# UbiquityRobotics/fiducials

Hardware: NVIDIA H100
Metric: frames/sec 1920x1080 (detect+pose) (higher is better)
Workload: dtype u8/i32 (threshold, contours), f32/f64 (sub-pixel, pose, map)

## Files before the change

fiducials_b200/csrc/fid_map.cu:

```cuda
#include <cuda_runtime.h>
#include <stdio.h>
#include <string.h>

#include <algorithm>
#include <vector>

#include "../../include/fiducials_b200.h"
#include "slam.cuh"

using namespace fid;



#include "fid_map_internal.h"

struct SeqArgs {
    MapState* state;
    MapEntry* entries;
    uint32_t* links;
    int cap, links_wpr;
    int32_t* hash;
    int hash_size;
    int n_instances, n_msgs;
    const int32_t* offsets;
    const Obs* obs;
    double* var_scratch;
    int* slot_scratch;
    const Twv* tf;
    int have_base_cam, have_cam_base;
    double weighting_scale, systematic_error;
    int use_area;
    RobotPose* robot;
};

__global__ void k_map_sequence(const SeqArgs a) {
    const int inst = blockIdx.x * blockDim.x + threadIdx.x;
    if (inst >= a.n_instances) return;
    MapState st = a.state[inst];
    MapEntry* e = a.entries + (size_t)inst * a.cap;
    uint32_t* links = a.links ? a.links + (size_t)inst * a.cap * a.links_wpr : nullptr;
    const int32_t* off = a.offsets + (size_t)inst * (a.n_msgs + 1);
    MapHash hash{a.hash + (size_t)inst * 2 * a.hash_size, a.hash + (size_t)inst * 2 * a.hash_size + a.hash_size, a.hash_size};
    for (int k = 0; k < a.n_msgs; k++) {
        RobotPose rp;
        map_update(st, e, links, a.obs + off[k], off[k + 1] - off[k], a.have_base_cam ? &a.tf[0] : nullptr, a.have_cam_base ? &a.tf[1] : nullptr, a.weighting_scale,
                   a.use_area, a.systematic_error, &rp, &hash, a.var_scratch + off[k], a.slot_scratch + off[k]);
        if (a.robot) a.robot[(size_t)inst * a.n_msgs + k] = rp;
    }
    a.state[inst] = st;
}

__global__ void k_map_export(const MapState* state, const MapEntry* entries, int cap, int inst, fid_map_record* table) {
    const MapState st = state[inst];
    const MapEntry* e = entries + (size_t)inst * cap;
    for (int i = threadIdx.x; i < cap; i += blockDim.x) {
        fid_map_record r;
        r.fiducial_id = -1;
        r.num_obs = 0;
        r.t[0] = r.t[1] = r.t[2] = 0;
        r.q[0] = r.q[1] = r.q[2] = 0;
        r.q[3] = 1;
        r.variance = 0;
        if (i < st.n) {
            int rank = 0;
            for (int j = 0; j < st.n; j++) rank += e[j].id < e[i].id ? 1 : 0;
            r.fiducial_id = e[i].id;
            r.num_obs = e[i].num_obs;
            r.t[0] = e[i].pose.t[0];
            r.t[1] = e[i].pose.t[1];
            r.t[2] = e[i].pose.t[2];
            m_to_q(e[i].pose.R, r.q);
            r.variance = e[i].pose.var;
            table[rank] = r;
        }
        if (i >= st.n) table[i] = r;
    }
}

#define MERGE_MAX_KEYS 4096
__device__ __forceinline__ int merge_key(int id) { return id < 0 ? 0x7fffffff : id; }
__device__ int table_find(const fid_map_record* tab, int cap, int id) {
    int lo = 0, hi = cap;
    while (lo < hi) {
        const int mid = (lo + hi) >> 1;
        if (merge_key(tab[mid].fiducial_id) < id)
            lo = mid + 1;
        else
            hi = mid;
    }
    return (lo < cap && tab[lo].fiducial_id == id) ? lo : -1;
}
__device__ void merge_fold(const fid_map_record* tables, int cap, int n_tables, int t0, int i0, MapEntry* out) {
    const fid_map_record& r0 = tables[(size_t)t0 * cap + i0];
    Twv pose;
    q_to_m(r0.q, pose.R);
    pose.t[0] = r0.t[0];
    pose.t[1] = r0.t[1];
    pose.t[2] = r0.t[2];
    pose.var = r0.variance;
    int num = r0.num_obs;
    for (int t = t0 + 1; t < n_tables; t++) {
        const fid_map_record* tab = tables + (size_t)t * cap;
        const int j = table_find(tab, cap, r0.fiducial_id);
        if (j < 0) continue;
        num += tab[j].num_obs;
        if (pose.var == 0.0) continue;
        Twv other;
        q_to_m(tab[j].q, other.R);
        other.t[0] = tab[j].t[0];
        other.t[1] = tab[j].t[1];
        other.t[2] = tab[j].t[2];
        other.var = tab[j].variance;
        if (other.var == 0.0)
            pose = other;
        else
            twv_update(pose, other);
    }
    out->id = r0.fiducial_id;
    out->num_obs = num;
    out->pose = pose;
}

struct MergedHeader {
    int32_t n;
    int32_t overflow;
};

__global__ void __launch_bounds__(1024) k_map_merge_view(int cap, int n_tables, const fid_map_record* tables, MapEntry* merged, MergedHeader* hdr) {
    __shared__ unsigned long long keys[MERGE_MAX_KEYS];
    const int total = n_tables * cap;
    for (int e = threadIdx.x; e < MERGE_MAX_KEYS; e += blockDim.x) {
        unsigned long long k = ~0ull;
        if (e < total) {
            const int t = e / cap, i = e - t * cap;
            const int id = tables[e].fiducial_id;
            bool owner = id >= 0;
            for (int t2 = 0; owner && t2 < t; t2++) owner = table_find(tables + (size_t)t2 * cap, cap, id) < 0;
            if (owner) k = ((unsigned long long)(unsigned int)id << 32) | (unsigned int)e;
            (void)i;
        }
        keys[e] = k;
    }
    __syncthreads();
    for (int k = 2; k <= MERGE_MAX_KEYS; k <<= 1)
        for (int j = k >> 1; j > 0; j >>= 1) {
            for (int e = threadIdx.x; e < MERGE_MAX_KEYS; e += blockDim.x) {
                const int p = e ^ j;
                if (p > e) {
                    const unsigned long long a = keys[e], b = keys[p];
                    const bool up = (e & k) == 0;
                    if ((a > b) == up) {
                        keys[e] = b;
                        keys[p] = a;
                    }
                }
            }
            __syncthreads();
        }
    for (int e = threadIdx.x; e < MERGE_MAX_KEYS; e += blockDim.x) {
        const unsigned long long k = keys[e];
        const bool valid = k != ~0ull;
        if (valid && e < cap) {
            const int src = (int)(unsigned int)k;
            merge_fold(tables, cap, n_tables, src / cap, src % cap, &merged[e]);
        }
        const bool last = valid && (e + 1 == MERGE_MAX_KEYS || keys[e + 1] == ~0ull);
        if (last) {
            hdr->n = e + 1 < cap ? e + 1 : cap;
            hdr->overflow = e + 1 > cap ? 1 : 0;
        }
        if (e == 0 && !valid) {
            hdr->n = 0;
            hdr->overflow = 0;
        }
    }
}

__global__ void k_map_merge_view_serial(int cap, int n_tables, const fid_map_record* tables, MapEntry* merged, MergedHeader* hdr) {
    if (threadIdx.x != 0 || blockIdx.x != 0) return;
    int n = 0, overflow = 0;
    int last_id = -1;
    for (;;) {
        int best = 0x7fffffff, bt = -1, bi = -1;
        for (int t = 0; t < n_tables; t++) {
            const fid_map_record* tab = tables + (size_t)t * cap;
            int lo = 0, hi = cap;
            while (lo < hi) {
                const int mid = (lo + hi) >> 1;
                if (merge_key(tab[mid].fiducial_id) <= last_id)
                    lo = mid + 1;
                else
                    hi = mid;
            }
            if (lo < cap && tab[lo].fiducial_id >= 0 && tab[lo].fiducial_id < best) {
                best = tab[lo].fiducial_id;
                bt = t;
                bi = lo;
            }
        }
        if (bt < 0) break;
        if (n < cap)
            merge_fold(tables, cap, n_tables, bt, bi, &merged[n++]);
// ... 96 lines not shown
extern "C" int fid_map_clear(fid_map* m, int instance) {
    if (!m || instance < 0 || instance >= m->p.n_instances) return FID_ERR_INVALID_ARG;
    CK(cudaSetDevice(m->device));
    CK(cudaStreamSynchronize(m->stream));
    MapState st;
    CK(cudaMemcpy(&st, m->d_state + instance, sizeof(st), cudaMemcpyDeviceToHost));
    st.n = 0;
    st.initial_frame_num = st.frame_num;
    st.origin_fid = -1;
    st.initializing = 0;
    st.overflow = 0;
    st.hash_valid = 0;
    CK(cudaMemcpy(m->d_state + instance, &st, sizeof(st), cudaMemcpyHostToDevice));
    const size_t wpr = (m->p.max_fiducials + 31) / 32;
    CK(cudaMemset(m->d_links + (size_t)instance * m->p.max_fiducials * wpr, 0, sizeof(uint32_t) * (size_t)m->p.max_fiducials * wpr));
    return FID_OK;
}

extern "C" int fid_map_add_fiducial(fid_map* m, int instance, int fiducial_id, const fid_tf* T_mapBase) {
    if (!m || instance < 0 || instance >= m->p.n_instances || fiducial_id < 0) return FID_ERR_INVALID_ARG;
    CK(cudaSetDevice(m->device));
    CK(cudaStreamSynchronize(m->stream));
    MapState st;
    CK(cudaMemcpy(&st, m->d_state + instance, sizeof(st), cudaMemcpyDeviceToHost));
    st.fiducial_to_add = fiducial_id;
    st.add_have_map_base = T_mapBase ? 1 : 0;
    if (T_mapBase) {
        for (int k = 0; k < 3; k++) st.add_map_base[k] = T_mapBase->t[k];
        for (int k = 0; k < 4; k++) st.add_map_base[3 + k] = T_mapBase->q[k];
    }
    CK(cudaMemcpy(m->d_state + instance, &st, sizeof(st), cudaMemcpyHostToDevice));
    return FID_OK;
}

static void tf_to_twv(const fid_tf& t, Twv* o) {
    q_to_m(t.q, o->R);
    o->t[0] = t.t[0];
    o->t[1] = t.t[1];
    o->t[2] = t.t[2];
    o->var = 0.0;
}

extern "C" int fid_map_load(fid_map* m, int instance, int n, const fid_map_file_entry* entries) {
    if (!m || instance < 0 || instance >= m->p.n_instances || n < 0 || (n > 0 && !entries)) return FID_ERR_INVALID_ARG;
    CK(cudaSetDevice(m->device));
    CK(cudaStreamSynchronize(m->stream));
    MapState st;
    CK(cudaMemcpy(&st, m->d_state + instance, sizeof(st), cudaMemcpyDeviceToHost));
    std::vector<MapEntry> e(st.capacity);
    if (st.n) CK(cudaMemcpy(e.data(), m->d_entries + (size_t)instance * st.capacity, sizeof(MapEntry) * st.n, cudaMemcpyDeviceToHost));
    const int lcap = m->p.max_fiducials, lwpr = (lcap + 31) / 32;
    std::vector<uint32_t> rows;
    bool rows_dirty = false;
    const double d2r = 3.14159265358979323846 / 180.0;
    for (int i = 0; i < n; i++) {
        const double hr = entries[i].roll_deg * d2r * 0.5, hp = entries[i].pitch_deg * d2r * 0.5, hy = entries[i].yaw_deg * d2r * 0.5;
        const double cy = cos(hy), sy = sin(hy), cp = cos(hp), sp = sin(hp), cr = cos(hr), sr = sin(hr);
        const double q[4] = {sr * cp * cy - cr * sp * sy, cr * sp * cy + sr * cp * sy, cr * cp * sy - sr * sp * cy, cr * cp * cy + sr * sp * sy};
        int slot = -1;
        for (int j = 0; j < st.n; j++)
            if (e[j].id == entries[i].fiducial_id) slot = j;
        if (slot < 0) {
            if (st.n >= st.capacity) return FID_ERR_CAPACITY;
            slot = st.n++;
        } else {
            if (rows.empty()) {
                rows.resize((size_t)lcap * lwpr);
                CK(cudaMemcpy(rows.data(), m->d_links + (size_t)instance * lcap * lwpr, sizeof(uint32_t) * rows.size(), cudaMemcpyDeviceToHost));
            }
            for (int w = 0; w < lwpr; w++) rows[(size_t)slot * lwpr + w] = 0;
            for (int j = 0; j < lcap; j++) rows[(size_t)j * lwpr + (slot >> 5)] &= ~(1u << (slot & 31));
            rows_dirty = true;
        }
        e[slot].id = entries[i].fiducial_id;
        e[slot].num_obs = entries[i].num_obs;
        q_to_m(q, e[slot].pose.R);
        e[slot].pose.t[0] = entries[i].x;
        e[slot].pose.t[1] = entries[i].y;
        e[slot].pose.t[2] = entries[i].z;
        e[slot].pose.var = entries[i].variance;
    }
    st.hash_valid = 0;
    if (st.n) CK(cudaMemcpy(m->d_entries + (size_t)instance * st.capacity, e.data(), sizeof(MapEntry) * st.n, cudaMemcpyHostToDevice));
    if (rows_dirty) CK(cudaMemcpy(m->d_links + (size_t)instance * lcap * lwpr, rows.data(), sizeof(uint32_t) * rows.size(), cudaMemcpyHostToDevice));
    CK(cudaMemcpy(m->d_state + instance, &st, sizeof(st), cudaMemcpyHostToDevice));
    return FID_OK;
}

template <class T>
static int ensure(T** p, size_t* cap, size_t need) {
    if (need <= *cap) return FID_OK;
    if (*p) cudaFree(*p);
    *p = nullptr;
    *cap = 0;
    const size_t n = std::max<size_t>(need, 1024);
    if (cudaMalloc((void**)p, sizeof(T) * n) != cudaSuccess) {
        cudaGetLastError();
        return FID_ERR_NO_MEMORY;
    }
    *cap = n;
    return FID_OK;
}

static int run_sequence(fid_map* m, int inst_lo, int n_inst, int n_msgs, const int32_t* offsets, const fid_transform* obs, const fid_tf* T_baseCam,
                        const fid_tf* T_camBase, fid_robot_pose* robot, bool async = false) {
    CK(cudaSetDevice(m->device));
    CK(cudaStreamSynchronize(m->stream));
    const size_t n_off = (size_t)n_inst * (n_msgs + 1);
    size_t total_obs = 0;
    for (size_t i = 0; i < n_off; i++) total_obs = std::max<size_t>(total_obs, (size_t)offsets[i]);
    int rc;
    if ((rc = ensure(&m->d_obs, &m->obs_cap, total_obs + 1)) != FID_OK || (rc = ensure(&m->d_var_scratch, &m->var_cap, total_obs + 1)) != FID_OK ||
        (rc = ensure(&m->d_slot_scratch, &m->slot_cap, total_obs + 1)) != FID_OK || (rc = ensure(&m->d_offsets, &m->off_cap, n_off)) != FID_OK ||
        (rc = ensure(&m->d_robot, &m->robot_cap, (size_t)n_inst * n_msgs + 1)) != FID_OK)
        return rc;
    std::vector<Obs> ho(total_obs);
    for (size_t i = 0; i < total_obs; i++) {
        ho[i].id = obs[i].fiducial_id;
        ho[i].pad = 0;
        for (int k = 0; k < 3; k++) ho[i].t[k] = obs[i].translation[k];
        for (int k = 0; k < 4; k++) ho[i].q[k] = obs[i].rotation[k];
        ho[i].object_error = obs[i].object_error;
        ho[i].area = obs[i].fiducial_area;
    }
    if (total_obs) CK(cudaMemcpyAsync(m->d_obs, ho.data(), sizeof(Obs) * total_obs, cudaMemcpyHostToDevice, m->stream));
    CK(cudaMemcpyAsync(m->d_offsets, offsets, sizeof(int32_t) * n_off, cudaMemcpyHostToDevice, m->stream));
    Twv tf[2];
    memset(tf, 0, sizeof(tf));
    if (T_baseCam) tf_to_twv(*T_baseCam, &tf[0]);
    if (T_camBase) tf_to_twv(*T_camBase, &tf[1]);
    CK(cudaMemcpyAsync(m->d_tf, tf, sizeof(tf), cudaMemcpyHostToDevice, m->stream));
    SeqArgs a{};
    const int cap = m->p.max_fiducials;
    a.state = m->d_state + inst_lo;
    a.entries = m->d_entries + (size_t)inst_lo * cap;
    a.links_wpr = (cap + 31) / 32;
    a.links = m->d_links + (size_t)inst_lo * cap * a.links_wpr;
    a.cap = cap;
    a.hash = m->d_hash + (size_t)inst_lo * 2 * m->hash_size;
    a.hash_size = m->hash_size;
    a.n_instances = n_inst;
    a.n_msgs = n_msgs;
    a.offsets = m->d_offsets;
    a.obs = m->d_obs;
    a.var_scratch = m->d_var_scratch;
    a.slot_scratch = m->d_slot_scratch;
    a.tf = m->d_tf;
    a.have_base_cam = T_baseCam ? 1 : 0;
    a.have_cam_base = T_camBase ? 1 : 0;
    a.weighting_scale = m->p.weighting_scale;
    a.systematic_error = m->p.systematic_error;
    a.use_area = m->p.use_fiducial_area_as_weight;
    a.robot = m->d_robot;
    k_map_sequence<<<(n_inst + 31) / 32, 32, 0, m->stream>>>(a);
    CK(cudaGetLastError());
    if (async) return FID_OK;
    std::vector<RobotPose> hr((size_t)n_inst * n_msgs);
    CK(cudaMemcpyAsync(hr.data(), m->d_robot, sizeof(RobotPose) * hr.size(), cudaMemcpyDeviceToHost, m->stream));
    CK(cudaStreamSynchronize(m->stream));
    if (robot)
        for (size_t i = 0; i < hr.size(); i++) {
            robot[i].valid = hr[i].valid;
            robot[i].n_estimates = hr[i].n_estimates;
            for (int k = 0; k < 3; k++) robot[i].t[k] = hr[i].t[k];
            for (int k = 0; k < 4; k++) robot[i].q[k] = hr[i].q[k];
            robot[i].variance = hr[i].var;
        }
    return FID_OK;
}

extern "C" int fid_map_update(fid_map* m, int instance, int n_obs, const fid_transform* obs, const fid_tf* T_baseCam, const fid_tf* T_camBase, fid_robot_pose* robot) {
    if (!m || instance < 0 || instance >= m->p.n_instances || n_obs < 0 || (n_obs > 0 && !obs)) return FID_ERR_INVALID_ARG;
    const int32_t off[2] = {0, n_obs};
    return run_sequence(m, instance, 1, 1, off, obs, T_baseCam, T_camBase, robot);
}

extern "C" int fid_map_update_sequence(fid_map* m, int n_msgs, const int32_t* offsets, const fid_transform* obs, const fid_tf* T_baseCam, const fid_tf* T_camBase,
                                       fid_robot_pose* robot) {
    if (!m || n_msgs < 1 || !offsets) return FID_ERR_INVALID_ARG;
    const size_t n_off = (size_t)m->p.n_instances * (n_msgs + 1);
    for (size_t i = 0; i + 1 < n_off; i++) {
        if ((i + 1) % (n_msgs + 1) == 0) continue;
        const int d = offsets[i + 1] - offsets[i];
        if (d < 0) return FID_ERR_INVALID_ARG;
    }
    return run_sequence(m, 0, m->p.n_instances, n_msgs, offsets, obs, T_baseCam, T_camBase, robot);
}

static int update_frames_impl(fid_map* m, int instance, int n_frames, const int32_t* counts, const fid_transform* transforms, int max_markers, const fid_tf* T_baseCam,
                              const fid_tf* T_camBase, fid_robot_pose* last_robot, bool async) {
    if (!m || instance < 0 || instance >= m->p.n_instances || n_frames < 1 || !counts || !transforms || max_markers < 1) return FID_ERR_INVALID_ARG;
    std::vector<int32_t> off((size_t)n_frames + 1, 0);
    std::vector<fid_transform> flat;
    for (int f = 0; f < n_frames; f++) {
        const int c = std::min(std::max(counts[f], 0), max_markers);
        off[f] = (int32_t)flat.size();
        flat.insert(flat.end(), transforms + (size_t)f * max_markers, transforms + (size_t)f * max_markers + c);
    }
    off[n_frames] = (int32_t)flat.size();
    std::vector<fid_robot_pose> robots((size_t)n_frames);
    fid_transform dummy{};
    const int rc = run_sequence(m, instance, 1, n_frames, off.data(), flat.empty() ? &dummy : flat.data(), T_baseCam, T_camBase, async ? nullptr : robots.data(), async);
    if (rc == FID_OK && last_robot && !async) *last_robot = robots[(size_t)n_frames - 1];
    return rc;
}

extern "C" int fid_map_update_frames(fid_map* m, int instance, int n_frames, const int32_t* counts, const fid_transform* transforms, int max_markers, const fid_tf* T_baseCam,
                                     const fid_tf* T_camBase, fid_robot_pose* last_robot) {
    return update_frames_impl(m, instance, n_frames, counts, transforms, max_markers, T_baseCam, T_camBase, last_robot, false);
}
extern "C" int fid_map_update_frames_async(fid_map* m, int instance, int n_frames, const int32_t* counts, const fid_transform* transforms, int max_markers,
                                           const fid_tf* T_baseCam, const fid_tf* T_camBase) {
    return update_frames_impl(m, instance, n_frames, counts, transforms, max_markers, T_baseCam, T_camBase, nullptr, true);
}
extern "C" int fid_map_sync(fid_map* m) {
    if (!m) return FID_ERR_INVALID_ARG;
    CK(cudaSetDevice(m->device));
    CK(cudaStreamSynchronize(m->stream));
    return FID_OK;
}

extern "C" int fid_map_entries(fid_map* m, int instance, int max_entries, int* n, fid_map_entry* entries) {
    if (!m || instance < 0 || instance >= m->p.n_instances || !n) return FID_ERR_INVALID_ARG;
    CK(cudaSetDevice(m->device));
    CK(cudaStreamSynchronize(m->stream));
    MapState st;
    CK(cudaMemcpy(&st, m->d_state + instance, sizeof(st), cudaMemcpyDeviceToHost));
    std::vector<MapEntry> e(st.n);
    if (st.n) CK(cudaMemcpy(e.data(), m->d_entries + (size_t)instance * st.capacity, sizeof(MapEntry) * st.n, cudaMemcpyDeviceToHost));
    std::sort(e.begin(), e.end(), [](const MapEntry& a, const MapEntry& b) { return a.id < b.id; });
    *n = st.n;
    if (st.n > max_entries) return FID_ERR_CAPACITY;
    for (int i = 0; i < st.n && entries; i++) {
        entries[i].fiducial_id = e[i].id;
        entries[i].num_obs = e[i].num_obs;
        entries[i].x = e[i].pose.t[0];
        entries[i].y = e[i].pose.t[1];
        entries[i].z = e[i].pose.t[2];
        get_rpy(e[i].pose.R, &entries[i].rx, &entries[i].ry, &entries[i].rz);
        entries[i].variance = e[i].pose.var;
    }
    return st.overflow ? FID_ERR_CAPACITY : FID_OK;
}

extern "C" int fid_map_links(fid_map* m, int instance, int max_pairs, int* n_pairs, int32_t* pairs) {
    if (!m || instance < 0 || instance >= m->p.n_instances || !n_pairs || max_pairs < 0) return FID_ERR_INVALID_ARG;
    CK(cudaSetDevice(m->device));
    CK(cudaStreamSynchronize(m->stream));
    MapState st;
    CK(cudaMemcpy(&st, m->d_state + instance, sizeof(st), cudaMemcpyDeviceToHost));
    const int cap = m->p.max_fiducials, wpr = (cap + 31) / 32;
    std::vector<MapEntry> e(st.n);
    std::vector<uint32_t> rows((size_t)st.n * wpr);
    if (st.n) {
        CK(cudaMemcpy(e.data(), m->d_entries + (size_t)instance * st.capacity, sizeof(MapEntry) * st.n, cudaMemcpyDeviceToHost));
        CK(cudaMemcpy(rows.data(), m->d_links + (size_t)instance * cap * wpr, sizeof(uint32_t) * rows.size(), cudaMemcpyDeviceToHost));
    }
    std::vector<std::pair<int32_t, int32_t>> out;
    for (int i = 0; i < st.n; i++)
        for (int j = 0; j < st.n; j++)
            if ((rows[(size_t)i * wpr + (j >> 5)] >> (j & 31)) & 1u) out.emplace_back(e[i].id, e[j].id);
    std::sort(out.begin(), out.end());
    *n_pairs = (int)out.size();
    if ((int)out.size() > max_pairs) return FID_ERR_CAPACITY;
    for (size_t k = 0; k < out.size() && pairs; k++) {
        pairs[2 * k] = out[k].first;
        pairs[2 * k + 1] = out[k].second;
    }
    return FID_OK;
}

extern "C" int fid_map_add_links(fid_map* m, int instance, int n_pairs, const int32_t* pairs) {
    if (!m || instance < 0 || instance >= m->p.n_instances || n_pairs < 0 || (n_pairs > 0 && !pairs)) return FID_ERR_INVALID_ARG;
    if (n_pairs == 0) return FID_OK;
    CK(cudaSetDevice(m->device));
    CK(cudaStreamSynchronize(m->stream));
    MapState st;
    CK(cudaMemcpy(&st, m->d_state + instance, sizeof(st), cudaMemcpyDeviceToHost));
    const int cap = m->p.max_fiducials, wpr = (cap + 31) / 32;
    std::vector<MapEntry> e(st.n);
    std::vector<uint32_t> rows((size_t)st.n * wpr);
    if (!st.n) return FID_OK;
    CK(cudaMemcpy(e.data(), m->d_entries + (size_t)instance * st.capacity, sizeof(MapEntry) * st.n, cudaMemcpyDeviceToHost));
    CK(cudaMemcpy(rows.data(), m->d_links + (size_t)instance * cap * wpr, sizeof(uint32_t) * rows.size(), cudaMemcpyDeviceToHost));
    auto slot_of = [&](int32_t id) {
        for (int i = 0; i < st.n; i++)
            if (e[i].id == id) return i;
        return -1;
    };
    for (int k = 0; k < n_pairs; k++) {
        const int i = slot_of(pairs[2 * k]), j = slot_of(pairs[2 * k + 1]);
        if (i >= 0 && j >= 0) rows[(size_t)i * wpr + (j >> 5)] |= 1u << (j & 31);
    }
    CK(cudaMemcpy(m->d_links + (size_t)instance * cap * wpr, rows.data(), sizeof(uint32_t) * rows.size(), cudaMemcpyHostToDevice));
    return FID_OK;
}

static int launch_export(fid_map* m, int instance, fid_map_record* dst) {
    k_map_export<<<1, 256, 0, m->stream>>>(m->d_state, m->d_entries, m->p.max_fiducials, instance, dst);
    CK(cudaGetLastError());
    return FID_OK;
}

extern "C" int fid_map_export_device(fid_map* m, int instance, void** device_table, size_t* bytes) {
    if (!m || instance < 0 || instance >= m->p.n_instances || !device_table || !bytes) return FID_ERR_INVALID_ARG;
    CK(cudaSetDevice(m->device));
    fid_map_record* tab = m->d_export + (size_t)instance * m->p.max_fiducials;
// ... 92 lines not shown
```

fiducials_b200/csrc/slam.cuh:

```cuda
#pragma once
#include "common.cuh"

namespace fid {

struct Twv {
    double R[9];
    double t[3];
    double var;
};

FID_HD void q_to_m(const double q[4], double m[9]) {
    const double x = q[0], y = q[1], z = q[2], w = q[3];
    const double d = x * x + y * y + z * z + w * w;
    const double s = 2.0 / d;
    const double xs = x * s, ys = y * s, zs = z * s;
    const double wx = w * xs, wy = w * ys, wz = w * zs;
    const double xx = x * xs, xy = x * ys, xz = x * zs;
    const double yy = y * ys, yz = y * zs, zz = z * zs;
    m[0] = 1.0 - (yy + zz);
    m[1] = xy - wz;
    m[2] = xz + wy;
    m[3] = xy + wz;
    m[4] = 1.0 - (xx + zz);
    m[5] = yz - wx;
    m[6] = xz - wy;
    m[7] = yz + wx;
    m[8] = 1.0 - (xx + yy);
}

FID_HD void m_to_q(const double m[9], double q[4]) {
    const double tr = m[0] + m[4] + m[8];
    if (tr > 0.0) {
        double s = sqrt(tr + 1.0);
        q[3] = s * 0.5;
        s = 0.5 / s;
        q[0] = (m[7] - m[5]) * s;
        q[1] = (m[2] - m[6]) * s;
        q[2] = (m[3] - m[1]) * s;
    } else {
        const int i = m[0] < m[4] ? (m[4] < m[8] ? 2 : 1) : (m[0] < m[8] ? 2 : 0);
        const int j = (i + 1) % 3, k = (i + 2) % 3;
        double s = sqrt(m[i * 3 + i] - m[j * 3 + j] - m[k * 3 + k] + 1.0);
        q[i] = s * 0.5;
        s = 0.5 / s;
        q[3] = (m[k * 3 + j] - m[j * 3 + k]) * s;
        q[j] = (m[j * 3 + i] + m[i * 3 + j]) * s;
        q[k] = (m[k * 3 + i] + m[i * 3 + k]) * s;
    }
}

FID_HD void get_rpy(const double m[9], double* roll, double* pitch, double* yaw) {
    if (fabs(m[6]) >= 1.0) {
        *yaw = 0.0;
        const double delta = atan2(m[7], m[8]);
        if (m[6] < 0) {
            *pitch = 3.14159265358979323846 / 2.0;
            *roll = delta;
        } else {
            *pitch = -3.14159265358979323846 / 2.0;
            *roll = delta;
        }
        return;
    }
    *pitch = -asin(m[6]);
    const double c = cos(*pitch);
    *roll = atan2(m[7] / c, m[8] / c);
    *yaw = atan2(m[3] / c, m[0] / c);
}

FID_HD Twv twv_mul(const Twv& a, const Twv& b) {
    Twv o;
    for (int i = 0; i < 3; i++) {
        for (int j = 0; j < 3; j++) o.R[i * 3 + j] = a.R[i * 3] * b.R[j] + a.R[i * 3 + 1] * b.R[3 + j] + a.R[i * 3 + 2] * b.R[6 + j];
        o.t[i] = (a.R[i * 3] * b.t[0] + a.R[i * 3 + 1] * b.t[1] + a.R[i * 3 + 2] * b.t[2]) + a.t[i];
    }
    o.var = a.var + b.var;
    return o;
}

FID_HD Twv twv_inverse(const Twv& a) {
    Twv o;
    for (int i = 0; i < 3; i++)
        for (int j = 0; j < 3; j++) o.R[i * 3 + j] = a.R[j * 3 + i];
    const double n[3] = {-a.t[0], -a.t[1], -a.t[2]};
    for (int i = 0; i < 3; i++) o.t[i] = o.R[i * 3] * n[0] + o.R[i * 3 + 1] * n[1] + o.R[i * 3 + 2] * n[2];
    o.var = a.var;
    return o;
}

FID_HD double prob_at_point(double x, double u, double var) {
    return (1.0 / (sqrt(var) * sqrt(2.0 * 3.14159265358979323846))) * exp(-((x - u) * (x - u)) / (2.0 * var));
}

FID_HD double normalize_david(double new_mean, double mean1, double var1, double mean2, double var2) {
    const double p1 = prob_at_point(new_mean, mean1, var1);
    const double p2 = prob_at_point(new_mean, mean2, var2);
    const double p = sqrt(p1 * p1 + p2 * p2);
    const double r = 1.0 / (p * sqrt(2.0 * 3.14159265358979323846));
    double nv = r * r;
    nv = nv < 1e3 ? nv : 1e3;
    nv = nv > 1e-8 ? nv : 1e-8;
    return nv;
}

FID_HD void twv_update(Twv& self, const Twv& n) {
    double q1[4], q2[4];
    m_to_q(self.R, q1);
    m_to_q(n.R, q2);
    const double v1 = self.var, v2 = n.var;
    const double p1[3] = {self.t[0], self.t[1], self.t[2]};
    const double k = v1 / (v1 + v2);
    for (int i = 0; i < 3; i++) self.t[i] = p1[i] + k * (n.t[i] - p1[i]);
    const double dot = q1[0] * q2[0] + q1[1] * q2[1] + q1[2] * q2[2] + q1[3] * q2[3];
    const double s = sqrt((q1[0] * q1[0] + q1[1] * q1[1] + q1[2] * q1[2] + q1[3] * q1[3]) * (q2[0] * q2[0] + q2[1] * q2[1] + q2[2] * q2[2] + q2[3] * q2[3]));
    double c = (dot < 0 ? -dot : dot) / s;
    c = c < -1.0 ? -1.0 : (c > 1.0 ? 1.0 : c);
    const double theta = acos(c);
    double q[4];
    if (theta != 0.0) {
        const double d = 1.0 / sin(theta);
        const double s0 = sin((1.0 - k) * theta), s1 = sin(k * theta);
        for (int i = 0; i < 4; i++) q[i] = dot < 0 ? (q1[i] * s0 + -q2[i] * s1) * d : (q1[i] * s0 + q2[i] * s1) * d;
    } else {
        for (int i = 0; i < 4; i++) q[i] = q1[i];
    }
    const double nrm = sqrt(q[0] * q[0] + q[1] * q[1] + q[2] * q[2] + q[3] * q[3]);
    for (int i = 0; i < 4; i++) q[i] /= nrm;
    q_to_m(q, self.R);
    const double d0 = n.t[0] - p1[0], d1 = n.t[1] - p1[1], d2 = n.t[2] - p1[2];
    const double mean2 = sqrt(d0 * d0 + d1 * d1 + d2 * d2);
    const double e0 = self.t[0] - p1[0], e1 = self.t[1] - p1[1], e2 = self.t[2] - p1[2];
    const double mean = sqrt(e0 * e0 + e1 * e1 + e2 * e2);
    self.var = normalize_david(mean, 0.0, v1, mean2, v2);
}

struct MapEntry {
    int32_t id;
    int32_t num_obs;
    Twv pose;
};

struct MapState {
    int32_t n;
    int32_t capacity;
    int32_t frame_num;
    int32_t initial_frame_num;
    int32_t origin_fid;
    int32_t initializing;
    int32_t read_only;
    int32_t overflow;
    int32_t hash_size;
    int32_t hash_valid;
    int32_t fiducial_to_add;
    int32_t add_have_map_base;
    double add_map_base[7];
};

struct MapHash {
    int32_t* keys;
    int32_t* vals;
    int32_t size;
};

FID_HD uint32_t map_hash_of(int id) { return (uint32_t)id * 2654435761u; }

FID_HD void map_hash_insert(const MapHash& h, int id, int slot) {
    uint32_t p = map_hash_of(id) & (uint32_t)(h.size - 1);
    while (h.keys[p] != 0 && h.keys[p] != id + 1) p = (p + 1) & (uint32_t)(h.size - 1);
    h.keys[p] = id + 1;
    h.vals[p] = slot;
}

FID_HD void map_hash_rebuild(const MapHash& h, const struct MapEntry* e, int n);

struct Obs {
    int32_t id;
    int32_t pad;
    double t[3];
    double q[4];
    double object_error;
    double area;
};

struct RobotPose {
    int32_t valid;
    int32_t n_estimates;
    double t[3];
    double q[4];
    double var;
};


FID_HD void map_hash_rebuild(const MapHash& h, const MapEntry* e, int n) {
    for (int i = 0; i < h.size; i++) h.keys[i] = 0;
    for (int i = 0; i < n; i++) map_hash_insert(h, e[i].id, i);
}

FID_HD int map_find(const MapState& st, const MapEntry* e, int id, const MapHash* h = nullptr) {
    if (h && h->size > 0) {
        uint32_t p = map_hash_of(id) & (uint32_t)(h->size - 1);
        while (h->keys[p] != 0) {
            if (h->keys[p] == id + 1) return h->vals[p];
            p = (p + 1) & (uint32_t)(h->size - 1);
        }
        return -1;
    }
    for (int i = 0; i < st.n; i++)
        if (e[i].id == id) return i;
    return -1;
}

FID_HD bool isnan3(const double t[3]) { return t[0] != t[0] || t[1] != t[1] || t[2] != t[2]; }

FID_HD Twv obs_cam_fid(const Obs& o, double weighting_scale, int use_area) {
    Twv t;
    q_to_m(o.q, t.R);
    t.t[0] = o.t[0];
    t.t[1] = o.t[1];
    t.t[2] = o.t[2];
    t.var = use_area ? weighting_scale / o.area : weighting_scale * o.object_error;
    return t;
}

FID_HD void map_update_core(MapState& st, MapEntry* e, uint32_t* links, const Obs* obs_in, int n_obs, const Twv* T_baseCam ,
                            const Twv* T_camBase , double weighting_scale, int use_area, double systematic_error, RobotPose* robot,
                            const MapHash* hash, double* var_scratch, int* slot_scratch) {
    if (hash && hash->size > 0 && !st.hash_valid) {
        map_hash_rebuild(*hash, e, st.n);
        st.hash_valid = 1;
    }
    robot->valid = 0;
    robot->n_estimates = 0;
    st.frame_num++;
    if (n_obs > 0 && st.n == 0) st.initializing = 1;
    if (st.initializing) {
        if (st.n == 0) {
            int idx = -1;
            double smallest = -1.0;
            for (int i = 0; i < n_obs; i++) {
                const double* ct = obs_in[i].t;
                const double d = ct[0] * ct[0] + ct[1] * ct[1] + ct[2] * ct[2];
                if (smallest < 0 || d < smallest) {
                    smallest = d;
                    idx = i;
                }
            }
            if (idx >= 0 && st.capacity > 0) {
                st.origin_fid = obs_in[idx].id;
                const Twv cf = obs_cam_fid(obs_in[idx], weighting_scale, use_area);
                Twv T = cf;
                if (T_baseCam) {
                    T = twv_mul(*T_baseCam, cf);
                    T.var = cf.var;
                }
                e[0].id = obs_in[idx].id;
                e[0].num_obs = 0;
                e[0].pose = T;
                st.n = 1;
                if (hash && hash->size > 0) map_hash_insert(*hash, obs_in[idx].id, 0);
            } else if (idx >= 0) {
                st.overflow = 1;
            }
        } else {
            for (int i = 0; i < n_obs; i++) {
                if (obs_in[i].id == st.origin_fid) {
                    const Twv cf = obs_cam_fid(obs_in[i], weighting_scale, use_area);
                    Twv T = cf;
                    if (T_baseCam) {
                        T = twv_mul(*T_baseCam, cf);
                        T.var = cf.var;
                    }
                    const int slot = map_find(st, e, st.origin_fid, hash);
                    if (slot >= 0) {
                        twv_update(e[slot].pose, T);
                        e[slot].num_obs++;
                    }
                    break;
                }
            }
        }
        if (st.frame_num - st.initial_frame_num > 10 && st.origin_fid != -1) {
            st.initializing = 0;
            const int slot = map_find(st, e, st.origin_fid, hash);
            if (slot >= 0) e[slot].pose.var = 0.0;
        }
        return;
    }
    if (n_obs == 0 || !T_baseCam) return;
    Twv camBase;
    if (T_camBase) {
        camBase = *T_camBase;
        camBase.var = 1.0;
    } else {
        for (int i = 0; i < 9; i++) camBase.R[i] = (i % 4 == 0) ? 1.0 : 0.0;
        camBase.t[0] = camBase.t[1] = camBase.t[2] = 0.0;
        camBase.var = 0.0;
    }
    Twv baseCam = *T_baseCam;
    baseCam.var = 1.0;
    int n_est = 0;
    Twv mapBase;
    for (int i = 0; i < n_obs; i++) {
        const Twv cf = obs_cam_fid(obs_in[i], weighting_scale, use_area);
        var_scratch[i] = cf.var;
        const int slot = map_find(st, e, obs_in[i].id, hash);
        if (slot < 0) continue;
        Twv fidCam = twv_inverse(cf);
        Twv p = twv_mul(e[slot].pose, fidCam);
        p = twv_mul(p, camBase);
        double roll, pitch, yaw;
        get_rpy(p.R, &roll, &pitch, &yaw);
        const double* c = cf.t;
        const double zr = p.t[2] / c[2];
        const double s1 = (zr * zr) * (c[0] * c[0] + c[1] * c[1]);
        const double len2 = p.t[0] * p.t[0] + p.t[1] * p.t[1] + p.t[2] * p.t[2];
        const double sr = sin(roll), spt = sin(pitch);
        const double s2 = len2 * (sr * sr);
        const double s3 = len2 * (spt * spt);
        p.var = s1 + s2 + s3 + systematic_error;
        var_scratch[i] = p.var;
        if (isnan3(p.t)) continue;
        if (n_est == 0) {
            mapBase = p;
        } else {
            twv_update(mapBase, p);
        }
        n_est++;
    }
    if (n_est == 0) return;
    robot->valid = 1;
    robot->n_estimates = n_est;
    robot->t[0] = mapBase.t[0];
    robot->t[1] = mapBase.t[1];
    robot->t[2] = mapBase.t[2];
    m_to_q(mapBase.R, robot->q);
    robot->var = mapBase.var;
    const Twv mapCam = twv_mul(mapBase, baseCam);
    if (n_obs > 1 && !st.read_only) {
        for (int i = 0; i < n_obs; i++) {
            Twv cf = obs_cam_fid(obs_in[i], weighting_scale, use_area);
            cf.var = var_scratch[i];
            const Twv mapFid = twv_mul(mapCam, cf);
            if (isnan3(mapFid.t)) continue;
            int slot = map_find(st, e, obs_in[i].id, hash);
            if (slot < 0) {
                if (st.n >= st.capacity) {
                    st.overflow = 1;
                    continue;
                }
                slot = st.n++;
                e[slot].id = obs_in[i].id;
                e[slot].num_obs = 0;
                e[slot].pose = mapFid;
                if (hash && hash->size > 0) map_hash_insert(*hash, obs_in[i].id, slot);
            }
            if (e[slot].pose.var != 0) {
                twv_update(e[slot].pose, mapFid);
                e[slot].num_obs += 2;
            }
        }
        if (links) {
            const int wpr = (st.capacity + 31) / 32;
            int* slots = slot_scratch;
            for (int i = 0; i < n_obs; i++) slots[i] = map_find(st, e, obs_in[i].id, hash);
            for (int i = 0; i < n_obs; i++) {
                if (slots[i] < 0) continue;
                for (int j = 0; j < n_obs; j++) {
                    if (obs_in[j].id == obs_in[i].id || slots[j] < 0) continue;
                    links[(size_t)slots[i] * wpr + (slots[j] >> 5)] |= 1u << (slots[j] & 31);
                }
            }
        }
    }
}

FID_HD void map_handle_add_fiducial(MapState& st, MapEntry* e, const Obs* obs_in, int n_obs, const Twv* T_baseCam, double weighting_scale, int use_area,
                                    const MapHash* hash) {
    if (st.fiducial_to_add == -1) return;
    if (map_find(st, e, st.fiducial_to_add, hash) >= 0) {
        st.fiducial_to_add = -1;
        return;
    }
    for (int i = 0; i < n_obs; i++) {
        if (obs_in[i].id != st.fiducial_to_add) continue;
        Twv T = obs_cam_fid(obs_in[i], weighting_scale, use_area);
        const double var = T.var;
        if (T_baseCam) T = twv_mul(*T_baseCam, T);
        if (st.add_have_map_base) {
            Twv mb;
            q_to_m(st.add_map_base + 3, mb.R);
            mb.t[0] = st.add_map_base[0];
            mb.t[1] = st.add_map_base[1];
            mb.t[2] = st.add_map_base[2];
            mb.var = 0.0;
            T = twv_mul(mb, T);
        }
        T.var = var;
        if (st.n >= st.capacity) {
            st.overflow = 1;
        } else {
            const int slot = st.n++;
            e[slot].id = obs_in[i].id;
            e[slot].num_obs = 0;
            e[slot].pose = T;
            if (hash && hash->size > 0) map_hash_insert(*hash, obs_in[i].id, slot);
            const int os = st.origin_fid != -1 ? map_find(st, e, st.origin_fid, hash) : -1;
            if (os >= 0) e[os].pose.var = 0.0;
        }
        st.initializing = 0;
        st.fiducial_to_add = -1;
        return;
    }
}

FID_HD void map_update(MapState& st, MapEntry* e, uint32_t* links, const Obs* obs_in, int n_obs, const Twv* T_baseCam ,
                       const Twv* T_camBase , double weighting_scale, int use_area, double systematic_error, RobotPose* robot,
                       const MapHash* hash, double* var_scratch, int* slot_scratch) {
    map_update_core(st, e, links, obs_in, n_obs, T_baseCam, T_camBase, weighting_scale, use_area, systematic_error, robot, hash, var_scratch, slot_scratch);
    map_handle_add_fiducial(st, e, obs_in, n_obs, T_baseCam, weighting_scale, use_area, hash);
}

}
```

Measured before the change: 10840.

## Parallelize map update across a warp per instance with shared state

Switches the map sequence kernel from one thread per map instance to one warp per instance. Per-observation pose estimates, map insertions and link-matrix updates are computed in parallel across lanes, using ballot, match_any and shuffles, and state and link masks are kept in shared memory. The pose fusion is split so quaternions are computed in parallel and only the serial fusion step stays ordered. This trades added warp synchronization and shared-memory use for parallelism on frames with many observations, and the reordered updates risk small numerical differences.

```diff
diff --git a/fiducials_b200/csrc/fid_map.cu b/fiducials_b200/csrc/fid_map.cu
--- a/fiducials_b200/csrc/fid_map.cu
+++ b/fiducials_b200/csrc/fid_map.cu
@@ -31,23 +31,203 @@
     double weighting_scale, systematic_error;
     int use_area;
     RobotPose* robot;
+    int shared_per_warp;
 };
 
+constexpr unsigned FULL_MASK = 0xffffffffu;
+constexpr int MAP_WARPS_PER_BLOCK = 4;
+constexpr size_t MAP_STATE_SHARED = (sizeof(MapState) + 15) & ~(size_t)15;
+
+static size_t map_shared_per_warp(int wpr) { return MAP_STATE_SHARED + ((sizeof(uint32_t) * (2 * (size_t)wpr + 1) + 15) & ~(size_t)15); }
+
+__device__ __forceinline__ double shfl_d(double v, int src) { return __shfl_sync(FULL_MASK, v, src); }
+
+__device__ void warp_update(MapState& st, MapEntry* e, uint32_t* links, int wpr, const Obs* obs, int n_obs, const Twv& T_baseCam, const Twv* T_camBase,
+                            double weighting_scale, int use_area, double systematic_error, RobotPose& robot, const MapHash& hash, double* var_scratch,
+                            int* slot_scratch, uint32_t* mask, uint32_t* words, int* n_words) {
+    const int lane = threadIdx.x & 31;
+    const uint32_t lanes_below = (1u << lane) - 1u;
+    const Twv camBase = map_cam_base(T_camBase);
+    int n_est = 0;
+    Twv mapBase = {};
+    for (int base = 0; base < n_obs; base += 32) {
+        const int i = base + lane;
+        bool valid = false;
+        Twv p = {};
+        double q[4] = {0.0, 0.0, 0.0, 1.0};
+        if (i < n_obs) {
+            const Twv cf = obs_cam_fid(obs[i], weighting_scale, use_area);
+            double var = cf.var;
+            const int slot = map_find(st, e, obs[i].id, &hash);
+            if (slot >= 0) {
+                p = map_pose_estimate(cf, e[slot].pose, camBase, systematic_error);
+                var = p.var;
+                valid = !isnan3(p.t);
+                m_to_q(p.R, q);
+            }
+            var_scratch[i] = var;
+        }
+        for (uint32_t vm = __ballot_sync(FULL_MASK, valid); vm; vm &= vm - 1) {
+            const int b = __ffs(vm) - 1;
+            const double t[3] = {shfl_d(p.t[0], b), shfl_d(p.t[1], b), shfl_d(p.t[2], b)};
+            const double v = shfl_d(p.var, b);
+            if (n_est == 0) {
+                for (int j = 0; j < 9; j++) mapBase.R[j] = shfl_d(p.R[j], b);
+                for (int j = 0; j < 3; j++) mapBase.t[j] = t[j];
+                mapBase.var = v;
+            } else {
+                const double qb[4] = {shfl_d(q[0], b), shfl_d(q[1], b), shfl_d(q[2], b), shfl_d(q[3], b)};
+                twv_update_q(mapBase, t, v, qb);
+            }
+            n_est++;
+        }
+    }
+    if (n_est == 0) return;
+    robot.valid = 1;
+    robot.n_estimates = n_est;
+    robot.t[0] = mapBase.t[0];
+    robot.t[1] = mapBase.t[1];
+    robot.t[2] = mapBase.t[2];
+    m_to_q(mapBase.R, robot.q);
+    robot.var = mapBase.var;
+    if (n_obs <= 1 || st.read_only) return;
+    Twv baseCam = T_baseCam;
+    baseCam.var = 1.0;
+    const Twv mapCam = twv_mul(mapBase, baseCam);
+    for (int base = 0; base < n_obs; base += 32) {
+        const int i = base + lane;
+        Twv mapFid = {};
+        int id = 0;
+        bool ok = false;
+        if (i < n_obs) {
+            Twv cf = obs_cam_fid(obs[i], weighting_scale, use_area);
+            cf.var = var_scratch[i];
+            mapFid = twv_mul(mapCam, cf);
+            id = obs[i].id;
+            ok = !isnan3(mapFid.t);
+        }
+        const uint32_t group = __match_any_sync(FULL_MASK, ok ? (unsigned long long)(uint32_t)id : (1ull << 32) | (unsigned)lane);
+        const int leader = __ffs(group) - 1;
+        const int rank = __popc(group & lanes_below);
+        int slot = ok && lane == leader ? map_find(st, e, id, &hash) : -1;
+        const bool fresh = ok && lane == leader && slot < 0;
+        const uint32_t fresh_mask = __ballot_sync(FULL_MASK, fresh);
+        const int n0 = st.n, room = st.capacity - n0;
+        if (fresh) {
+            const int r = __popc(fresh_mask & lanes_below);
+            slot = r < room ? n0 + r : -1;
+        }
+        slot = __shfl_sync(FULL_MASK, slot, leader);
+        const int n_fresh = __popc(fresh_mask);
+        const int n_new = n_fresh < room ? n_fresh : room;
+        __syncwarp();
+        int r = 0;
+        for (uint32_t fm = fresh_mask; fm && r < n_new; fm &= fm - 1, r++) {
+            const int idb = __shfl_sync(FULL_MASK, id, __ffs(fm) - 1);
+            if (lane == 0) map_hash_insert(hash, idb, n0 + r);
+        }
+        if (lane == 0) {
+            st.n = n0 + n_new;
+            if (n_fresh > room) st.overflow = 1;
+        }
+        if (fresh && slot >= 0) {
+            e[slot].id = id;
+            e[slot].num_obs = 0;
+            e[slot].pose = mapFid;
+        }
+        const int rounds = __reduce_max_sync(FULL_MASK, ok && slot >= 0 ? (unsigned)__popc(group) : 0u);
+        for (int k = 0; k < rounds; k++) {
+            __syncwarp();
+            if (ok && slot >= 0 && rank == k && e[slot].pose.var != 0) {
+                twv_update(e[slot].pose, mapFid);
+                e[slot].num_obs += 2;
+            }
+        }
+        __syncwarp();
+    }
+    if (!links) return;
+    for (int w = lane; w < wpr; w += 32) mask[w] = 0u;
+    if (lane == 0) *n_words = 0;
+    __syncwarp();
+    for (int i = lane; i < n_obs; i += 32) {
+        const int slot = map_find(st, e, obs[i].id, &hash);
+        slot_scratch[i] = slot;
+        if (slot >= 0) {
+            const uint32_t old = atomicOr(&mask[slot >> 5], 1u << (slot & 31));
+            if (old == 0u) words[atomicAdd(n_words, 1)] = (uint32_t)(slot >> 5);
+        }
+    }
+    __syncwarp();
+    const int nw = *n_words;
+    for (int base = 0; base < n_obs; base += 32) {
+        const int i = base + lane;
+        const int slot = i < n_obs ? slot_scratch[i] : -1;
+        const uint32_t same = __match_any_sync(FULL_MASK, slot);
+        if (slot >= 0 && lane == __ffs(same) - 1) {
+            uint32_t* row = links + (size_t)slot * wpr;
+            for (int k = 0; k < nw; k++) {
+                const int w = (int)words[k];
+                const uint32_t m = w == (slot >> 5) ? mask[w] & ~(1u << (slot & 31)) : mask[w];
+                if (m) row[w] |= m;
+            }
+        }
+        __syncwarp();
+    }
+}
+
 __global__ void k_map_sequence(const SeqArgs a) {
-    const int inst = blockIdx.x * blockDim.x + threadIdx.x;
+    extern __shared__ __align__(16) unsigned char map_shared[];
+    const int warp = threadIdx.x >> 5, lane = threadIdx.x & 31;
+    const int inst = blockIdx.x * (blockDim.x >> 5) + warp;
     if (inst >= a.n_instances) return;
-    MapState st = a.state[inst];
+    unsigned char* mine = map_shared + (size_t)warp * a.shared_per_warp;
+    MapState& st = *reinterpret_cast<MapState*>(mine);
+    uint32_t* mask = reinterpret_cast<uint32_t*>(mine + MAP_STATE_SHARED);
+    uint32_t* words = mask + a.links_wpr;
+    int* n_words = reinterpret_cast<int*>(words + a.links_wpr);
+    if (lane == 0) st = a.state[inst];
     MapEntry* e = a.entries + (size_t)inst * a.cap;
     uint32_t* links = a.links ? a.links + (size_t)inst * a.cap * a.links_wpr : nullptr;
     const int32_t* off = a.offsets + (size_t)inst * (a.n_msgs + 1);
-    MapHash hash{a.hash + (size_t)inst * 2 * a.hash_size, a.hash + (size_t)inst * 2 * a.hash_size + a.hash_size, a.hash_size};
+    const MapHash hash{a.hash + (size_t)inst * 2 * a.hash_size, a.hash + (size_t)inst * 2 * a.hash_size + a.hash_size, a.hash_size};
+    const Twv* T_baseCam = a.have_base_cam ? &a.tf[0] : nullptr;
+    const Twv* T_camBase = a.have_cam_base ? &a.tf[1] : nullptr;
+    __syncwarp();
     for (int k = 0; k < a.n_msgs; k++) {
+        const Obs* obs = a.obs + off[k];
+        const int n_obs = off[k + 1] - off[k];
+        if (!st.hash_valid) {
+            for (int i = lane; i < hash.size; i += 32) hash.keys[i] = 0;
+            __syncwarp();
+            if (lane == 0) {
+                for (int i = 0; i < st.n; i++) map_hash_insert(hash, e[i].id, i);
+                st.hash_valid = 1;
+            }
+            __syncwarp();
+        }
         RobotPose rp;
-        map_update(st, e, links, a.obs + off[k], off[k + 1] - off[k], a.have_base_cam ? &a.tf[0] : nullptr, a.have_cam_base ? &a.tf[1] : nullptr, a.weighting_scale,
-                   a.use_area, a.systematic_error, &rp, &hash, a.var_scratch + off[k], a.slot_scratch + off[k]);
-        if (a.robot) a.robot[(size_t)inst * a.n_msgs + k] = rp;
-    }
-    a.state[inst] = st;
+        rp.valid = 0;
+        rp.n_estimates = 0;
+        int initializing = 0;
+        if (lane == 0) {
+            st.frame_num++;
+            if (n_obs > 0 && st.n == 0) st.initializing = 1;
+            initializing = st.initializing;
+            if (initializing) map_auto_init(st, e, obs, n_obs, T_baseCam, a.weighting_scale, a.use_area, &hash);
+        }
+        initializing = __shfl_sync(FULL_MASK, initializing, 0);
+        __syncwarp();
+        if (!initializing && n_obs > 0 && T_baseCam)
+            warp_update(st, e, links, a.links_wpr, obs, n_obs, *T_baseCam, T_camBase, a.weighting_scale, a.use_area, a.systematic_error, rp, hash,
+                        a.var_scratch + off[k], a.slot_scratch + off[k], mask, words, n_words);
+        __syncwarp();
+        if (lane == 0) {
+            map_handle_add_fiducial(st, e, obs, n_obs, T_baseCam, a.weighting_scale, a.use_area, &hash);
+            if (a.robot) a.robot[(size_t)inst * a.n_msgs + k] = rp;
+        }
+        __syncwarp();
+    }
+    if (lane == 0) a.state[inst] = st;
 }
 
 __global__ void k_map_export(const MapState* state, const MapEntry* entries, int cap, int inst, fid_map_record* table) {
@@ -450,7 +630,10 @@
     a.systematic_error = m->p.systematic_error;
     a.use_area = m->p.use_fiducial_area_as_weight;
     a.robot = m->d_robot;
-    k_map_sequence<<<(n_inst + 31) / 32, 32, 0, m->stream>>>(a);
+    const size_t per_warp = map_shared_per_warp(a.links_wpr);
+    a.shared_per_warp = (int)per_warp;
+    const int wpb = std::max(1, std::min({MAP_WARPS_PER_BLOCK, n_inst, (int)((48 << 10) / per_warp)}));
+    k_map_sequence<<<(n_inst + wpb - 1) / wpb, 32 * wpb, per_warp * wpb, m->stream>>>(a);
     CK(cudaGetLastError());
     if (async) return FID_OK;
     std::vector<RobotPose> hr((size_t)n_inst * n_msgs);
diff --git a/fiducials_b200/csrc/slam.cuh b/fiducials_b200/csrc/slam.cuh
--- a/fiducials_b200/csrc/slam.cuh
+++ b/fiducials_b200/csrc/slam.cuh
@@ -103,14 +103,13 @@
     return nv;
 }
 
-FID_HD void twv_update(Twv& self, const Twv& n) {
-    double q1[4], q2[4];
+FID_HD void twv_update_q(Twv& self, const double nt[3], double nvar, const double q2[4]) {
+    double q1[4];
     m_to_q(self.R, q1);
-    m_to_q(n.R, q2);
-    const double v1 = self.var, v2 = n.var;
+    const double v1 = self.var, v2 = nvar;
     const double p1[3] = {self.t[0], self.t[1], self.t[2]};
     const double k = v1 / (v1 + v2);
-    for (int i = 0; i < 3; i++) self.t[i] = p1[i] + k * (n.t[i] - p1[i]);
+    for (int i = 0; i < 3; i++) self.t[i] = p1[i] + k * (nt[i] - p1[i]);
     const double dot = q1[0] * q2[0] + q1[1] * q2[1] + q1[2] * q2[2] + q1[3] * q2[3];
     const double s = sqrt((q1[0] * q1[0] + q1[1] * q1[1] + q1[2] * q1[2] + q1[3] * q1[3]) * (q2[0] * q2[0] + q2[1] * q2[1] + q2[2] * q2[2] + q2[3] * q2[3]));
     double c = (dot < 0 ? -dot : dot) / s;
@@ -127,11 +126,17 @@
     const double nrm = sqrt(q[0] * q[0] + q[1] * q[1] + q[2] * q[2] + q[3] * q[3]);
     for (int i = 0; i < 4; i++) q[i] /= nrm;
     q_to_m(q, self.R);
-    const double d0 = n.t[0] - p1[0], d1 = n.t[1] - p1[1], d2 = n.t[2] - p1[2];
+    const double d0 = nt[0] - p1[0], d1 = nt[1] - p1[1], d2 = nt[2] - p1[2];
     const double mean2 = sqrt(d0 * d0 + d1 * d1 + d2 * d2);
     const double e0 = self.t[0] - p1[0], e1 = self.t[1] - p1[1], e2 = self.t[2] - p1[2];
     const double mean = sqrt(e0 * e0 + e1 * e1 + e2 * e2);
     self.var = normalize_david(mean, 0.0, v1, mean2, v2);
+}
+
+FID_HD void twv_update(Twv& self, const Twv& n) {
+    double q2[4];
+    m_to_q(n.R, q2);
+    twv_update_q(self, n.t, n.var, q2);
 }
 
 struct MapEntry {
@@ -222,71 +227,60 @@
     return t;
 }
 
-FID_HD void map_update_core(MapState& st, MapEntry* e, uint32_t* links, const Obs* obs_in, int n_obs, const Twv* T_baseCam ,
-                            const Twv* T_camBase , double weighting_scale, int use_area, double systematic_error, RobotPose* robot,
-                            const MapHash* hash, double* var_scratch, int* slot_scratch) {
-    if (hash && hash->size > 0 && !st.hash_valid) {
-        map_hash_rebuild(*hash, e, st.n);
-        st.hash_valid = 1;
-    }
-    robot->valid = 0;
-    robot->n_estimates = 0;
-    st.frame_num++;
-    if (n_obs > 0 && st.n == 0) st.initializing = 1;
-    if (st.initializing) {
-        if (st.n == 0) {
-            int idx = -1;
-            double smallest = -1.0;
-            for (int i = 0; i < n_obs; i++) {
-                const double* ct = obs_in[i].t;
-                const double d = ct[0] * ct[0] + ct[1] * ct[1] + ct[2] * ct[2];
-                if (smallest < 0 || d < smallest) {
-                    smallest = d;
-                    idx = i;
-                }
-            }
-            if (idx >= 0 && st.capacity > 0) {
-                st.origin_fid = obs_in[idx].id;
-                const Twv cf = obs_cam_fid(obs_in[idx], weighting_scale, use_area);
+FID_HD void map_auto_init(MapState& st, MapEntry* e, const Obs* obs_in, int n_obs, const Twv* T_baseCam, double weighting_scale, int use_area, const MapHash* hash) {
+    if (st.n == 0) {
+        int idx = -1;
+        double smallest = -1.0;
+        for (int i = 0; i < n_obs; i++) {
+            const double* ct = obs_in[i].t;
+            const double d = ct[0] * ct[0] + ct[1] * ct[1] + ct[2] * ct[2];
+            if (smallest < 0 || d < smallest) {
+                smallest = d;
+                idx = i;
+            }
+        }
+        if (idx >= 0 && st.capacity > 0) {
+            st.origin_fid = obs_in[idx].id;
+            const Twv cf = obs_cam_fid(obs_in[idx], weighting_scale, use_area);
+            Twv T = cf;
+            if (T_baseCam) {
+                T = twv_mul(*T_baseCam, cf);
+                T.var = cf.var;
+            }
+            e[0].id = obs_in[idx].id;
+            e[0].num_obs = 0;
+            e[0].pose = T;
+            st.n = 1;
+            if (hash && hash->size > 0) map_hash_insert(*hash, obs_in[idx].id, 0);
+        } else if (idx >= 0) {
+            st.overflow = 1;
+        }
+    } else {
+        for (int i = 0; i < n_obs; i++) {
+            if (obs_in[i].id == st.origin_fid) {
+                const Twv cf = obs_cam_fid(obs_in[i], weighting_scale, use_area);
                 Twv T = cf;
                 if (T_baseCam) {
                     T = twv_mul(*T_baseCam, cf);
                     T.var = cf.var;
                 }
-                e[0].id = obs_in[idx].id;
-                e[0].num_obs = 0;
-                e[0].pose = T;
-                st.n = 1;
-                if (hash && hash->size > 0) map_hash_insert(*hash, obs_in[idx].id, 0);
-            } else if (idx >= 0) {
-                st.overflow = 1;
-            }
-        } else {
-            for (int i = 0; i < n_obs; i++) {
-                if (obs_in[i].id == st.origin_fid) {
-                    const Twv cf = obs_cam_fid(obs_in[i], weighting_scale, use_area);
-                    Twv T = cf;
-                    if (T_baseCam) {
-                        T = twv_mul(*T_baseCam, cf);
-                        T.var = cf.var;
-                    }
-                    const int slot = map_find(st, e, st.origin_fid, hash);
-                    if (slot >= 0) {
-                        twv_update(e[slot].pose, T);
-                        e[slot].num_obs++;
-                    }
-                    break;
+                const int slot = map_find(st, e, st.origin_fid, hash);
+                if (slot >= 0) {
+                    twv_update(e[slot].pose, T);
+                    e[slot].num_obs++;
                 }
-            }
-        }
-        if (st.frame_num - st.initial_frame_num > 10 && st.origin_fid != -1) {
-            st.initializing = 0;
-            const int slot = map_find(st, e, st.origin_fid, hash);
-            if (slot >= 0) e[slot].pose.var = 0.0;
-        }
-        return;
-    }
-    if (n_obs == 0 || !T_baseCam) return;
+                break;
+            }
+        }
+    }
+    if (st.frame_num - st.initial_frame_num > 10 && st.origin_fid != -1) {
+        st.initializing = 0;
+        const int slot = map_find(st, e, st.origin_fid, hash);
+        if (slot >= 0) e[slot].pose.var = 0.0;
+    }
+}
+
+FID_HD Twv map_cam_base(const Twv* T_camBase ) {
     Twv camBase;
     if (T_camBase) {
         camBase = *T_camBase;
@@ -296,6 +290,43 @@
         camBase.t[0] = camBase.t[1] = camBase.t[2] = 0.0;
         camBase.var = 0.0;
     }
+    return camBase;
+}
+
+FID_HD Twv map_pose_estimate(const Twv& cf, const Twv& fid_pose, const Twv& camBase, double systematic_error) {
+    Twv fidCam = twv_inverse(cf);
+    Twv p = twv_mul(fid_pose, fidCam);
+    p = twv_mul(p, camBase);
+    double roll, pitch, yaw;
+    get_rpy(p.R, &roll, &pitch, &yaw);
+    const double* c = cf.t;
+    const double zr = p.t[2] / c[2];
+    const double s1 = (zr * zr) * (c[0] * c[0] + c[1] * c[1]);
+    const double len2 = p.t[0] * p.t[0] + p.t[1] * p.t[1] + p.t[2] * p.t[2];
+    const double sr = sin(roll), spt = sin(pitch);
+    const double s2 = len2 * (sr * sr);
+    const double s3 = len2 * (spt * spt);
+    p.var = s1 + s2 + s3 + systematic_error;
+    return p;
+}
+
+FID_HD void map_update_core(MapState& st, MapEntry* e, uint32_t* links, const Obs* obs_in, int n_obs, const Twv* T_baseCam ,
+                            const Twv* T_camBase , double weighting_scale, int use_area, double systematic_error, RobotPose* robot,
+                            const MapHash* hash, double* var_scratch, int* slot_scratch) {
+    if (hash && hash->size > 0 && !st.hash_valid) {
+        map_hash_rebuild(*hash, e, st.n);
+        st.hash_valid = 1;
+    }
+    robot->valid = 0;
+    robot->n_estimates = 0;
+    st.frame_num++;
+    if (n_obs > 0 && st.n == 0) st.initializing = 1;
+    if (st.initializing) {
+        map_auto_init(st, e, obs_in, n_obs, T_baseCam, weighting_scale, use_area, hash);
+        return;
+    }
+    if (n_obs == 0 || !T_baseCam) return;
+    const Twv camBase = map_cam_base(T_camBase);
     Twv baseCam = *T_baseCam;
     baseCam.var = 1.0;
     int n_est = 0;
@@ -305,19 +336,7 @@
         var_scratch[i] = cf.var;
         const int slot = map_find(st, e, obs_in[i].id, hash);
         if (slot < 0) continue;
-        Twv fidCam = twv_inverse(cf);
-        Twv p = twv_mul(e[slot].pose, fidCam);
-        p = twv_mul(p, camBase);
-        double roll, pitch, yaw;
-        get_rpy(p.R, &roll, &pitch, &yaw);
-        const double* c = cf.t;
-        const double zr = p.t[2] / c[2];
-        const double s1 = (zr * zr) * (c[0] * c[0] + c[1] * c[1]);
-        const double len2 = p.t[0] * p.t[0] + p.t[1] * p.t[1] + p.t[2] * p.t[2];
-        const double sr = sin(roll), spt = sin(pitch);
-        const double s2 = len2 * (sr * sr);
-        const double s3 = len2 * (spt * spt);
-        p.var = s1 + s2 + s3 + systematic_error;
+        const Twv p = map_pose_estimate(cf, e[slot].pose, camBase, systematic_error);
         var_scratch[i] = p.var;
         if (isnan3(p.t)) continue;
         if (n_est == 0) {
```

After: 10930 (median of 6 runs). About the same (+0.8%).
